# google/telluride_decoding

Hardware: AMD Instinct MI355X
Metric: TRF-fit samples/sec (higher is better)
Workload: dtype f32 (every product as 3 float16 products of a 2-piece split on the f16 MFMA, f32 accumulate, f64 slab sums; f64 solve)

## Files before the change

telluride_decoding_amd/csrc/lagcov.hip:

```cpp
#include <cstdlib>
#include <cstring>

#include "lag_common.h"

namespace {

constexpr int kTile = 128;
constexpr int kTileG = 64;
constexpr int kNpfU = 10;
constexpr int kNpfU2 = 13;
constexpr int kNpfG = 9;
constexpr int kLagsPerWg = 8;
constexpr int kHalo = 8;
constexpr size_t kLagcovScratchCap = size_t(256) << 20;

__device__ __forceinline__ int xcd_remap(int bid, int nwg) {
  const int q = nwg >> 3, r = nwg & 7;
  const int xcd = bid & 7, within = bid >> 3;
  const int base = xcd < r ? xcd * (q + 1) : r * (q + 1) + (xcd - r) * q;
  return base + within;
}

struct RowWindow {
  const float* base;
// ... 57 lines not shown
  v.y = (ok && c4 + 1 <= rw.last) ? v.y : 0.f;
  v.z = (ok && c4 + 2 <= rw.last) ? v.z : 0.f;
  v.w = (ok && c4 + 3 <= rw.last) ? v.w : 0.f;
  return v;
}

template <bool kUnified, int kTileT, int kNPF, bool kVec4>
__device__ __forceinline__ void prefetch_tile(const LagParams& p, const LagWork& w, long long ut,
                                              int e0, int rows, int cat, int cbt, int tid,
                                              float4 (&pf)[kNPF]) {
  const int c4 = (tid & 15) * 4;
  const int r0 = tid >> 4;
  if (kUnified) {
    const RowWindow rw = row_window(p.a, p.lda, w.a_row0, ut, w.a_valid, cat * 64, p.ca);
#pragma unroll
    for (int i = 0; i < kNPF; ++i) {
      const int r = r0 + 16 * i;
      pf[i] = load_row4<kVec4>(rw, r, r < rows, c4);
    }
  } else {
    const RowWindow ra = row_window(p.a, p.lda, w.a_row0, ut, w.a_valid, cat * 64, p.ca);
    const RowWindow rb = row_window(p.b, p.ldb, w.b_row0, ut + e0, w.b_valid, cbt * 64, p.cb);
    const long long a_left = w.u_end - ut;
    const int a_lim = (int)(a_left < kTileT ? a_left : kTileT);
#pragma unroll
    for (int i = 0; i < kNPF; ++i) {
      const int r = r0 + 16 * i;
      if (16 * i + 15 < kTileT)
        pf[i] = load_row4<kVec4>(ra, r, r < a_lim, c4);
      else
        pf[i] = load_row4<kVec4>(rb, r - kTileT, r < rows, c4);
    }
  }
}

template <bool kUnified, int kTileT, int kNPF>
__device__ __forceinline__ void store_tile(float* lds, const LagWork& w, long long ut,
                                           int ones_col, int tid, float4 (&pf)[kNPF]) {
  const int c4 = (tid & 15) * 4;
#pragma unroll
  for (int i = 0; i < kNPF; ++i) {
    const int r = (tid >> 4) + 16 * i;
    float4 v = pf[i];
    if (!kUnified && 16 * i + 15 < kTileT && ones_col >= c4 && ones_col < c4 + 4) {
      const long long u = ut + r;
      const float one = (u >= w.u_begin && u < w.u_end) ? 1.f : 0.f;
      if (ones_col == c4) v.x = one;
      else if (ones_col == c4 + 1) v.y = one;
      else if (ones_col == c4 + 2) v.z = one;
      else v.w = one;
    }
    *reinterpret_cast<float4*>(lds + r * 64 + c4) = v;
  }
}

template <int kTileT, bool kM2, bool kN2>
__device__ __forceinline__ void mfma_tile(const float* __restrict__ as,
                                          const float* __restrict__ bs, int wave, int lane, int nk,
                                          f32x16 (&acc)[2][2][2]) {
  const int lr = lane & 31, lk = lane >> 5;
  const float* ap = as + lk * 64 + lr;
  const float* bp = bs + (lk + 2 * wave) * 64 + lr;
  auto ld = [&](int kk, float (&o)[6]) {
    o[0] = ap[kk * 128];
    o[1] = kM2 ? ap[kk * 128 + 32] : 0.f;
    o[2] = bp[kk * 128];
    o[3] = kN2 ? bp[kk * 128 + 32] : 0.f;
    o[4] = bp[kk * 128 + 64];
    o[5] = kN2 ? bp[kk * 128 + 96] : 0.f;
  };
  auto mm = [&](const float (&o)[6]) {
#pragma unroll
    for (int le = 0; le < 2; ++le) {
      const float b0 = o[2 + 2 * le], b1 = o[3 + 2 * le];
      acc[le][0][0] = __builtin_amdgcn_mfma_f32_32x32x2f32(o[0], b0, acc[le][0][0], 0, 0, 0);
      if (kM2) acc[le][1][0] = __builtin_amdgcn_mfma_f32_32x32x2f32(o[1], b0, acc[le][1][0], 0, 0, 0);
      if (kN2) {
        acc[le][0][1] = __builtin_amdgcn_mfma_f32_32x32x2f32(o[0], b1, acc[le][0][1], 0, 0, 0);
        if (kM2) acc[le][1][1] = __builtin_amdgcn_mfma_f32_32x32x2f32(o[1], b1, acc[le][1][1], 0, 0, 0);
      }
    }
  };
  const int nfull = nk >> 1;
  float c[6], n[6];
  ld(0, c);
  int kk = 0;
  for (; kk + 1 < nfull; kk += 2) {
    ld(kk + 1, n);
    mm(c);
    ld(kk + 2 < nfull ? kk + 2 : kk + 1, c);
    mm(n);
  }
  if (kk < nfull) mm(c);
  if (nk & 1) {
    ld(nfull, c);
    if (lk) { c[0] = 0.f; c[1] = 0.f; }
    mm(c);
  }
}

template <int kTileT, bool kM2, bool kN2>
__device__ __forceinline__ void mfma_tile_few(const float* __restrict__ as,
                                              const float* __restrict__ bs, int wave, int lane,
                                              int nk, int g, int lg, f32x16 (&acc)[2][2][2]) {
  const int lr = lane & 31, lk = lane >> 5;
  const int s_phases = 8 >> lg;
  const int nfull = nk >> 1;
#pragma unroll
  for (int le = 0; le < 2; ++le) {
    const int slot = 2 * wave + le;
    const int lag = slot & (g - 1), phase = slot >> lg;
    const float* ap = as + lk * 64 + lr;
    const float* bp = bs + (lk + lag) * 64 + lr;
    auto step = [&](int kk, bool tail) {
      const bool live = !tail || lk == 0;
      const float a0 = live ? ap[kk * 128] : 0.f;
      const float a1 = (kM2 && live) ? ap[kk * 128 + 32] : 0.f;
      const float b0 = bp[kk * 128];
      acc[le][0][0] = __builtin_amdgcn_mfma_f32_32x32x2f32(a0, b0, acc[le][0][0], 0, 0, 0);
      if (kM2) acc[le][1][0] = __builtin_amdgcn_mfma_f32_32x32x2f32(a1, b0, acc[le][1][0], 0, 0, 0);
      if (kN2) {
        const float b1 = bp[kk * 128 + 32];
        acc[le][0][1] = __builtin_amdgcn_mfma_f32_32x32x2f32(a0, b1, acc[le][0][1], 0, 0, 0);
        if (kM2) acc[le][1][1] = __builtin_amdgcn_mfma_f32_32x32x2f32(a1, b1, acc[le][1][1], 0, 0, 0);
      }
    };
#pragma unroll 4
    for (int kk = phase; kk < nfull; kk += s_phases) step(kk, false);
    if ((nk & 1) && (nfull & (s_phases - 1)) == phase) step(nfull, true);
  }
}

template <bool kUnified, int kTileT, int kNPF, bool kVec4, bool kFew>
__global__ __launch_bounds__(kThreads, 2) void lagcov_mfma_kernel(LagParams p) {
  extern __shared__ __attribute__((aligned(16))) float lds[];

  const int tid = threadIdx.x;
  const int lane = tid & 63;
  const int wave = __builtin_amdgcn_readfirstlane(tid >> 6);

  int id = xcd_remap(blockIdx.x, gridDim.x);
  const int group = id % p.n_groups; id /= p.n_groups;
  const int cbt = id % p.n_cbt; id /= p.n_cbt;
  const int cat = id % p.n_cat; id /= p.n_cat;
  const LagWork w = p.works[id];
  const int e0 = p.e_min + group * (kFew ? p.lag_g : kLagsPerWg);

  const int rows = kUnified ? kTileT + kHalo + e0 : 2 * kTileT + kHalo;
  const float* as = lds;
  const float* bs = kUnified ? lds + e0 * 64 : lds + kTileT * 64;

  const int ca_eff = p.ca + p.a_ones;
  const bool m2 = ca_eff - cat * 64 > 32;
  const bool n2 = p.cb - cbt * 64 > 32;
  const int ones_col = p.a_ones ? p.ca - cat * 64 : -1;

  f32x16 acc[2][2][2];
#pragma unroll
  for (int i = 0; i < 2; ++i)
#pragma unroll
    for (int j = 0; j < 2; ++j)
#pragma unroll
      for (int k = 0; k < 2; ++k)
#pragma unroll
        for (int r = 0; r < 16; ++r) acc[i][j][k][r] = 0.f;

  float4 pf[kNPF];
  prefetch_tile<kUnified, kTileT, kNPF, kVec4>(p, w, w.u_begin, e0, rows, cat, cbt, tid, pf);
  store_tile<kUnified, kTileT, kNPF>(lds, w, w.u_begin, ones_col, tid, pf);
  __syncthreads();

  for (long long ut = w.u_begin; ut < w.u_end; ut += kTileT) {
    const bool more = ut + kTileT < w.u_end;
    if (more)
      prefetch_tile<kUnified, kTileT, kNPF, kVec4>(p, w, ut + kTileT, e0, rows, cat, cbt, tid,
                                                      pf);
    const long long left = w.u_end - ut;
    const int nk = (kUnified && left < kTileT) ? (int)left : kTileT;
    if (kFew) {
      if (m2) {
        if (n2) mfma_tile_few<kTileT, true, true>(as, bs, wave, lane, nk, p.lag_g, p.lag_lg, acc);
        else    mfma_tile_few<kTileT, true, false>(as, bs, wave, lane, nk, p.lag_g, p.lag_lg, acc);
      } else {
        if (n2) mfma_tile_few<kTileT, false, true>(as, bs, wave, lane, nk, p.lag_g, p.lag_lg, acc);
        else    mfma_tile_few<kTileT, false, false>(as, bs, wave, lane, nk, p.lag_g, p.lag_lg, acc);
      }
    } else if (m2) {
      if (n2) mfma_tile<kTileT, true, true>(as, bs, wave, lane, nk, acc);
      else    mfma_tile<kTileT, true, false>(as, bs, wave, lane, nk, acc);
    } else {
      if (n2) mfma_tile<kTileT, false, true>(as, bs, wave, lane, nk, acc);
      else    mfma_tile<kTileT, false, false>(as, bs, wave, lane, nk, acc);
    }
    if (more) {
      __syncthreads();
      store_tile<kUnified, kTileT, kNPF>(lds, w, ut + kTileT, ones_col, tid, pf);
      __syncthreads();
    }
  }

  const int lr = lane & 31, lk = lane >> 5;
  float* slab = p.partial + (size_t)id * p.e_pad * p.ca_pad * p.cb_pad;
#pragma unroll
  for (int le = 0; le < 2; ++le) {
    int e_idx = group * kLagsPerWg + 2 * wave + le;
    if (kFew) {
      const int slot = 2 * wave + le;
      e_idx = ((slot >> p.lag_lg) * p.n_groups + group) * p.lag_g + (slot & (p.lag_g - 1));
    }
    float* pe = slab + (size_t)e_idx * p.ca_pad * p.cb_pad;
#pragma unroll
    for (int m = 0; m < 2; ++m)
#pragma unroll
      for (int n = 0; n < 2; ++n)
#pragma unroll
        for (int r = 0; r < 16; ++r) {
          const int i = cat * 64 + m * 32 + (r & 3) + 8 * (r >> 2) + 4 * lk;
          const int j = cbt * 64 + n * 32 + lr;
          pe[(size_t)i * p.cb_pad + j] = acc[le][m][n][r];
        }
  }
}

constexpr int kBfTile = 128;
template <int kRowDw, int kPieces> struct BfGeom {
  static constexpr int kRows = kRowDw == 83 ? 160 : 192;
  static constexpr int kPieceDw = 64 * kRowDw;
  static constexpr size_t kLdsBytes =
      sizeof(unsigned) * (2 * kPieces * kPieceDw + (kPieces == 2 ? 2 * 2 * 96 + 8 * 1024 : 0));
};
constexpr int kBfThreads = 512;

typedef td_u32x4 u32x4;

__device__ __forceinline__ float comp4(const float4& v, int q) {
  return q == 0 ? v.x : q == 1 ? v.y : q == 2 ? v.z : v.w;
}

#define TD_KS_C0(r) "0"
#define TD_KS_C1(r) "%" #r
#define TD_KS_BODY(C, MASK_L, MASK_H, TAIL)                                              \
  "ds_read2_b32 v[224:225], %[bp0] offset0:%[o0] offset1:%[o1]\n"                        \
  "ds_read2_b32 v[226:227], %[bp0] offset0:%[o2] offset1:%[o3]\n"                        \
  "ds_read2_b32 v[228:229], %[bp0] offset0:%[o4] offset1:%[o5]\n"                        \
  "ds_read_b32 v230, %[bp0] offset:%[ob]\n"                                              \
  "ds_read2_b32 v[220:221], %[ap1] offset0:%[o0] offset1:%[o1]\n"                        \
  "ds_read2_b32 v[222:223], %[ap1] offset0:%[o2] offset1:%[o3]\n"                        \
  "ds_read2_b32 v[232:233], %[bp1] offset0:%[o0] offset1:%[o1]\n"                        \
  "ds_read2_b32 v[234:235], %[bp1] offset0:%[o2] offset1:%[o3]\n"                        \
  "ds_read2_b32 v[236:237], %[bp1] offset0:%[o4] offset1:%[o5]\n"                        \
  "ds_read_b32 v238, %[bp1] offset:%[ob]\n"                                              \
  "ds_read2_b32 v[216:217], %[ap0] offset0:%[o0] offset1:%[o1]\n"                        \
  "ds_read2_b32 v[218:219], %[ap0] offset0:%[o2] offset1:%[o3]\n"                        \
  "s_waitcnt lgkmcnt(6)\n"                                                               \
  MASK_L                                                                                 \
  "v_alignbit_b32 v240, v225, v224, 16\n"                                                \
  "v_alignbit_b32 v241, v226, v225, 16\n"                                                \
  "v_alignbit_b32 v242, v227, v226, 16\n"                                                \
  "v_alignbit_b32 v243, v228, v227, 16\n"                                                \
  "v_alignbit_b32 v244, v229, v228, 16\n"                                                \
  "v_alignbit_b32 v245, v230, v229, 16\n"                                                \
  "v_mfma_f32_32x32x16_f16 %0, v[220:223], v[224:227], " C(0) "\n"                       \
  "s_waitcnt lgkmcnt(0)\n"                                                               \
  MASK_H                                                                                 \
  "v_alignbit_b32 v248, v233, v232, 16\n"                                                \
  "v_alignbit_b32 v249, v234, v233, 16\n"                                                \
  "v_mfma_f32_32x32x16_f16 %1, v[220:223], v[240:243], " C(1) "\n"                       \
  "v_alignbit_b32 v250, v235, v234, 16\n"                                                \
  "v_alignbit_b32 v251, v236, v235, 16\n"                                                \
  "v_mfma_f32_32x32x16_f16 %2, v[220:223], v[226:229], " C(2) "\n"                       \
  "v_alignbit_b32 v252, v237, v236, 16\n"                                                \
  "v_alignbit_b32 v253, v238, v237, 16\n"                                                \
  "v_mfma_f32_32x32x16_f16 %3, v[220:223], v[242:245], " C(3) "\n"                       \
  "v_mfma_f32_32x32x16_f16 %0, v[216:219], v[232:235], %0\n"                             \
  "v_mfma_f32_32x32x16_f16 %1, v[216:219], v[248:251], %1\n"                             \
  "v_mfma_f32_32x32x16_f16 %2, v[216:219], v[234:237], %2\n"                             \
  "v_mfma_f32_32x32x16_f16 %3, v[216:219], v[250:253], %3\n"                             \
  "v_mfma_f32_32x32x16_f16 %0, v[216:219], v[224:227], %0\n"                             \
  "v_mfma_f32_32x32x16_f16 %1, v[216:219], v[240:243], %1\n"                             \
  "v_mfma_f32_32x32x16_f16 %2, v[216:219], v[226:229], %2\n"                             \
  "v_mfma_f32_32x32x16_f16 %3, v[216:219], v[242:245], %3\n"                             \
  TAIL
#define TD_KS_MASK_L                                                                     \
  "v_and_b32 v220, %[m0], v220\n" "v_and_b32 v221, %[m1], v221\n"                        \
  "v_and_b32 v222, %[m2], v222\n" "v_and_b32 v223, %[m3], v223\n"
#define TD_KS_MASK_H                                                                     \
  "v_and_b32 v216, %[m0], v216\n" "v_and_b32 v217, %[m1], v217\n"                        \
  "v_and_b32 v218, %[m2], v218\n" "v_and_b32 v219, %[m3], v219\n"
#define TD_KS_TAIL "s_nop 15\ns_nop 3\n"
#define TD_KS_INS                                                                        \
  [ap0] "v"(ap0), [ap1] "v"(ap1), [bp0] "v"(bp0), [bp1] "v"(bp1),                        \
  [o0] "n"(kOff), [o1] "n"(kOff + 1), [o2] "n"(kOff + 2), [o3] "n"(kOff + 3),            \
  [o4] "n"(kOff + 4), [o5] "n"(kOff + 5), [ob] "n"(4 * (kOff + 6)),                      \
  [m0] "v"(m0), [m1] "v"(m1), [m2] "v"(m2), [m3] "v"(m3)
#define TD_KS_CLOBBER                                                                    \
  "memory", "v216", "v217", "v218", "v219", "v220", "v221", "v222", "v223", "v224", "v225", "v226", "v227", \
  "v228", "v229", "v230", "v231", "v232", "v233", "v234", "v235", "v236", "v237", "v238", "v239", "v240",   \
  "v241", "v242", "v243", "v244", "v245", "v246", "v247", "v248", "v249", "v250", "v251", "v252", "v253",   \
  "v254", "v255"
#define TD_KS_ASM(OUT, C, ML, MH, TAIL)                                                  \
  asm volatile(TD_KS_BODY(C, ML, MH, TAIL)                                               \
               : OUT(acc[0]), OUT(acc[1]), OUT(acc[2]), OUT(acc[3]) : TD_KS_INS : TD_KS_CLOBBER)

__device__ __forceinline__ unsigned lds_addr(const unsigned* p) {
  return (unsigned)(size_t)(__attribute__((address_space(3))) const unsigned*)p;
}

template <bool kZero, bool kMask, bool kLast, int kOff>
__device__ __forceinline__ void bf_kstep_skip(unsigned ap0, unsigned ap1, unsigned bp0, unsigned bp1,
                                              const unsigned* a_mask, f32x16 (&acc)[4]) {
  unsigned m0 = 0, m1 = 0, m2 = 0, m3 = 0;
  if constexpr (kMask) { m0 = a_mask[0]; m1 = a_mask[1]; m2 = a_mask[2]; m3 = a_mask[3]; }
  if constexpr (kZero) {
    if constexpr (kMask) {
      if constexpr (kLast) TD_KS_ASM("=&v", TD_KS_C0, TD_KS_MASK_L, TD_KS_MASK_H, TD_KS_TAIL);
      else TD_KS_ASM("=&v", TD_KS_C0, TD_KS_MASK_L, TD_KS_MASK_H, "");
    } else {
      if constexpr (kLast) TD_KS_ASM("=&v", TD_KS_C0, "", "", TD_KS_TAIL);
      else TD_KS_ASM("=&v", TD_KS_C0, "", "", "");
    }
  } else {
    if constexpr (kMask) {
      if constexpr (kLast) TD_KS_ASM("+v", TD_KS_C1, TD_KS_MASK_L, TD_KS_MASK_H, TD_KS_TAIL);
      else TD_KS_ASM("+v", TD_KS_C1, TD_KS_MASK_L, TD_KS_MASK_H, "");
    } else {
      if constexpr (kLast) TD_KS_ASM("+v", TD_KS_C1, "", "", TD_KS_TAIL);
      else TD_KS_ASM("+v", TD_KS_C1, "", "", "");
    }
  }
}

template <bool kZero, int kBfPieceDw, bool kF16, bool kSkip = false, int kOff = 0, bool kLast = true>
__device__ __forceinline__ void bf_kstep(const unsigned* __restrict__ ap,
                                         const unsigned* __restrict__ bp,
                                         const unsigned* a_mask, f32x16 (&acc)[4]) {
  if constexpr (kSkip) {
    static_assert(kF16, "lags +0, +1, +4, +5: the float16 form");
    const unsigned a0 = lds_addr(ap), b0 = lds_addr(bp);
    if (a_mask) bf_kstep_skip<kZero, true, kLast, kOff>(a0, a0 + 4 * kBfPieceDw, b0, b0 + 4 * kBfPieceDw, a_mask, acc);
    else bf_kstep_skip<kZero, false, kLast, kOff>(a0, a0 + 4 * kBfPieceDw, b0, b0 + 4 * kBfPieceDw, a_mask, acc);
    return;
  }
  constexpr int kP = kF16 ? 2 : 3;
  u32x4 a[kP];
  unsigned d[kP][6];
#pragma unroll
  for (int pc = 0; pc < kP; ++pc) {
#pragma unroll
    for (int i = 0; i < 4; ++i) a[pc][i] = ap[pc * kBfPieceDw + i];
#pragma unroll
    for (int i = 0; i < 6; ++i) d[pc][i] = bp[pc * kBfPieceDw + i];
  }
  if (a_mask) {
#pragma unroll
    for (int pc = 0; pc < kP; ++pc)
#pragma unroll
      for (int i = 0; i < 4; ++i) a[pc][i] &= a_mask[i];
  }
  u32x4 b[4][kP];
#pragma unroll
  for (int pc = 0; pc < kP; ++pc)
#pragma unroll
    for (int i = 0; i < 4; ++i) {
      b[0][pc][i] = d[pc][i];
      b[1][pc][i] = __builtin_amdgcn_alignbit(d[pc][i + 1], d[pc][i], 16);
      b[2][pc][i] = d[pc][i + 1];
      b[3][pc][i] = __builtin_amdgcn_alignbit(d[pc][i + 2], d[pc][i + 1], 16);
    }
  f32x16 c[4];
#pragma unroll
  for (int r = 0; r < 4; ++r) {
    if (kZero) {
#pragma unroll
      for (int k = 0; k < 16; ++k) c[r][k] = 0.f;
    } else {
      c[r] = acc[r];
    }
  }
  if constexpr (kF16) {
    constexpr int pa[3] = {1, 0, 0}, pb[3] = {0, 1, 0};
#pragma unroll
    for (int t = 0; t < 3; ++t)
#pragma unroll
      for (int r = 0; r < 4; ++r) c[r] = td_mfma_f16(a[pa[t] % kP], b[r][pb[t] % kP], c[r]);
  } else {
    constexpr int pa[6] = {2, 0, 1, 1, 0, 0}, pb[6] = {0, 2, 1, 0, 1, 0};
#pragma unroll
    for (int t = 0; t < 6; ++t)
#pragma unroll
      for (int r = 0; r < 4; ++r) c[r] = td_mfma_bf16(a[pa[t] % kP], b[r][pb[t] % kP], c[r]);
  }
#pragma unroll
  for (int r = 0; r < 4; ++r) acc[r] = c[r];
}

template <int kFrom, int kTo, int kBfPieceDw, bool kF16, int kChain, bool kSkip = false>
__device__ __forceinline__ void bf_ksteps(const unsigned* __restrict__ ap,
                                          const unsigned* __restrict__ bp, f32x16 (&acc)[4],
                                          f32x16 (&total)[4]) {
  if constexpr (kSkip) {
    if constexpr (kFrom < kTo) {
      constexpr bool kLast = (kFrom + 1) % kChain == 0;
      bf_kstep<kFrom % kChain == 0, kBfPieceDw, kF16, true, 8 * kFrom, kLast>(ap, bp, nullptr, acc);
      if (kLast) {
#pragma unroll
        for (int r = 0; r < 4; ++r) total[r] += acc[r];
      }
      __builtin_amdgcn_sched_barrier(0);
      bf_ksteps<kFrom + 1, kTo, kBfPieceDw, kF16, kChain, true>(ap, bp, acc, total);
    }
    return;
  }
#pragma unroll
  for (int s = kFrom; s < kTo; ++s) {
    if (s % kChain == 0) bf_kstep<true, kBfPieceDw, kF16>(ap + 8 * s, bp + 8 * s, nullptr, acc);
    else                 bf_kstep<false, kBfPieceDw, kF16>(ap + 8 * s, bp + 8 * s, nullptr, acc);
    if ((s + 1) % kChain == 0) {
#pragma unroll
      for (int r = 0; r < 4; ++r) total[r] += acc[r];
    }
    __builtin_amdgcn_sched_barrier(0);
  }
}

template <bool kVec4, int kBfRowDw, bool kF16, bool kVirt = false, bool kKs = false>
__global__ __launch_bounds__(kBfThreads) void lagcov_split_kernel(LagParams p) {
  static_assert(!kVirt || kF16, "virtual images: the float16 form");
  static_assert(!kKs || kVirt, "shared tasks: virtual images");
  constexpr int kChain = 8;
  constexpr int kP = kF16 ? 2 : 3;
  extern __shared__ __attribute__((aligned(16))) unsigned ldsu[];
  constexpr int kBfRows = BfGeom<kBfRowDw, kP>::kRows;
  constexpr int kBfPieceDw = BfGeom<kBfRowDw, kP>::kPieceDw;

  const int tid = threadIdx.x;
  const int lane = tid & 63;
  const int wave = __builtin_amdgcn_readfirstlane(tid >> 6);
  int quad = wave & 1, mt = (wave >> 1) & 1, nt = wave >> 2;
  constexpr bool kSkip = kF16 && !kVirt;

  int id = xcd_remap(blockIdx.x, gridDim.x);
  const int group = id % p.n_groups; id /= p.n_groups;
  const int part = id;
  LagWork w = p.works[id];
  const int e0 = group * kLagsPerWg;
  int lag_off = e0 + (kSkip ? 2 : 4) * quad, out_lag = lag_off;
  bool active = true, a_ext = false;
  const VirtImage* img = nullptr;
  VirtSeg vs = {0, 0, 0};
  int kparts = 1, kq = 0;
  if constexpr (kVirt) {
    const VirtGroup* vg = p.vgroups + group;
    const VirtTask tk = vg->task[wave];
    img = p.vimgs + vg->image;
    mt = tk.mt; nt = tk.nt; lag_off = tk.lag0; out_lag = tk.out_lag;
    active = out_lag >= 0; a_ext = tk.a_ext != 0;
    if constexpr (kKs) {
      kparts = __builtin_amdgcn_readfirstlane((int)tk.kparts);
      kq = __builtin_amdgcn_readfirstlane((int)tk.kq);
    }
    vs = p.vsegs[id];
  }
  const int ksn = 8 / kparts, ks0 = kq * ksn;

  f32x16 total[4];
#pragma unroll
  for (int r = 0; r < 4; ++r)
#pragma unroll
    for (int k = 0; k < 16; ++k) total[r][k] = 0.f;

  const int c4 = (tid & 15) * 4, rg = tid >> 4;
  const bool has_tail = kBfRows == 192 || wave < 4;
  const bool early = wave < 4;
  float sc[4] = {1.f, 1.f, 1.f, 1.f};
  int vdesc[4] = {0, 0, 0, 0};
  if constexpr (kVirt) {
#pragma unroll
    for (int q = 0; q < 4; ++q) {
      const int k = kVec4 ? c4 + q : lane;
      vdesc[q] = (img->src[k] + 1) | (img->role[k] ? 0x100 : 0) | ((int)img->shift[k] << 16);
    }
  }
  constexpr int kVPairs = kBfRows / 16;
  auto v_src = [&](int q) { return (vdesc[q] & 0xff) - 1; };
  auto v_sh = [&](int q) { return vdesc[q] >> 16; };
  auto v_role = [&](int q) { return (vdesc[q] & 0x100) != 0; };
  if (kF16) {
#pragma unroll
    for (int q = 0; q < 4; ++q) {
      const int ch = kVirt ? v_src(q) : min(c4 + q, 63);
      const int k = ch >= 0 ? td_f16_scale_exp(td_chan_max_of(p.chan_max, ch)) : 0;
      sc[q] = __builtin_bit_cast(float, (unsigned)(127 + k) << 23);
      if (kVirt && ch < 0) sc[q] = 0.f;
    }
    if (blockIdx.x == 0 && tid < 128) {
      unsigned* all = const_cast<unsigned*>(p.chan_max);
      const unsigned m = td_chan_max_of(p.chan_max, tid);
      all[kChanShards * 128 + tid] = m;
      if (p.scale_out) p.scale_out[tid] = m;
    }
    if (p.zero_tab && blockIdx.x == (gridDim.x > 1 ? 1 : 0))
      for (int i = tid; i < kChanTab; i += kBfThreads) p.zero_tab[i] = 0u;
  }
  const bool never = false;
  float anchor_a = 0.f, anchor_b = 1.f;
  auto sched_anchor = [&](unsigned* dst) {
    if (!never || tid >= 160) return;
    reinterpret_cast<unsigned short*>(dst)[tid] = (unsigned short)(anchor_a * anchor_b);
  };
  float4 pf[6];
  auto interior = [&](long long ut) -> bool {
    return kVec4 && p.ca == 64 && ut >= 0 && ut + kBfRows <= w.a_valid;
  };
  auto vrange = [&](long long ut, int q, int& lo, int& hi) {
    const long long lim = 1 << 20;
    const long long a0 = -ut, b0 = w.a_valid - ut;
    const long long a1 = vs.seg_begin - ut, b1 = (vs.seg_end < w.a_valid ? vs.seg_end : w.a_valid) - ut;
    const int a0i = (int)(a0 < -lim ? -lim : (a0 > lim ? lim : a0)), b0i = (int)(b0 < -lim ? -lim : (b0 > lim ? lim : b0));
    const int a1i = (int)(a1 < -lim ? -lim : (a1 > lim ? lim : a1)), b1i = (int)(b1 < -lim ? -lim : (b1 > lim ? lim : b1));
    lo = (v_role(q) ? a1i : a0i) - v_sh(q);
    hi = (v_role(q) ? b1i : b0i) - v_sh(q);
    if (v_src(q) < 0) { lo = 0; hi = 0; }
  };
  int v_min_shift = 0, v_max_shift = 0;
  bool v_any_role1 = false;
  if constexpr (kVirt) { v_min_shift = img->min_shift; v_max_shift = img->max_shift; v_any_role1 = img->any_role1 != 0; }
  auto vinside = [&](long long ut) -> bool {
    const long long lo = v_any_role1 && vs.seg_begin > 0 ? vs.seg_begin : 0;
    const long long hi = v_any_role1 && vs.seg_end < w.a_valid ? vs.seg_end : w.a_valid;
    return ut + v_min_shift >= lo && ut + kBfRows + v_max_shift <= hi;
  };
  auto prefetch_to = [&](long long ut, float4 (&pfr)[6]) {
    if constexpr (kVirt) {
      if (vinside(ut)) {
        const int ld = (int)p.lda;
        const float* base = p.a + (w.a_row0 + ut) * p.lda;
        if (kVec4) {
          const int off = (4 * rg + v_sh(0)) * ld + (v_src(0) < 0 ? 0 : v_src(0));
#pragma unroll
          for (int s = 0; s < 4; ++s) pfr[s] = *reinterpret_cast<const float4*>(base + s * ld + off);
          if (has_tail) {
            const float* tb = base + kBfTile * ld;
            const int toff = off - 2 * rg * ld;
#pragma unroll
            for (int s = 0; s < 2; ++s) pfr[4 + s] = *reinterpret_cast<const float4*>(tb + s * ld + toff);
          }
        } else {
          const int off = (2 * wave + v_sh(0)) * ld + (v_src(0) < 0 ? 0 : v_src(0));
          float* pv = reinterpret_cast<float*>(&pfr[0]);
#pragma unroll
          for (int j = 0; j < kVPairs; ++j) {
            pv[2 * j] = (base + 16 * j * ld)[off];
            pv[2 * j + 1] = (base + (16 * j + 1) * ld)[off];
          }
        }
        return;
      }
      const float* base = p.a + (w.a_row0 + ut) * p.lda;
      const int ld = (int)p.lda;
      const long long l0 = -ut, h0 = w.a_valid - 1 - ut, lim = 1 << 20;
      const int rlo = (int)(l0 < -lim ? -lim : (l0 > lim ? lim : l0));
      const int rhi = (int)(h0 < -lim ? -lim : (h0 > lim ? lim : h0));
      if (kVec4) {
        const int src = v_src(0) < 0 ? 0 : v_src(0), sh = v_sh(0);
#pragma unroll
        for (int s = 0; s < 4; ++s) {
          const int rc = max(rlo, min(4 * rg + s + sh, rhi));
          pfr[s] = *reinterpret_cast<const float4*>(base + rc * ld + src);
        }
        if (has_tail) {
#pragma unroll
          for (int s = 0; s < 2; ++s) {
            const int rc = max(rlo, min(kBfTile + 2 * rg + s + sh, rhi));
            pfr[4 + s] = *reinterpret_cast<const float4*>(base + rc * ld + src);
          }
        }
      } else {
        const int src = v_src(0) < 0 ? 0 : v_src(0), sh = v_sh(0);
        float* pv = reinterpret_cast<float*>(&pfr[0]);
#pragma unroll
        for (int j = 0; j < 2 * kVPairs; ++j) {
          const int r = 16 * (j >> 1) + 2 * wave + (j & 1);
          const int rc = max(rlo, min(r + sh, rhi));
          pv[j] = base[rc * ld + src];
        }
      }
      return;
    }
    if (interior(ut)) {
      const float* base = p.a + (w.a_row0 + ut) * p.lda + c4;
      const int ld = (int)p.lda;
#pragma unroll
      for (int s = 0; s < 4; ++s)
        pfr[s] = *reinterpret_cast<const float4*>(base + (4 * rg + s) * ld);
      if (has_tail) {
#pragma unroll
        for (int s = 0; s < 2; ++s)
          pfr[4 + s] = *reinterpret_cast<const float4*>(base + (kBfTile + 2 * rg + s) * ld);
      }
      return;
    }
    const RowWindow rw = row_window(p.a, p.lda, w.a_row0, ut, w.a_valid, 0, p.ca);
#pragma unroll
    for (int s = 0; s < 4; ++s) pfr[s] = load_row4_raw<kVec4>(rw, 4 * rg + s, c4);
    if (has_tail) {
#pragma unroll
      for (int s = 0; s < 2; ++s) pfr[4 + s] = load_row4_raw<kVec4>(rw, kBfTile + 2 * rg + s, c4);
    }
  };
  auto prefetch = [&](long long ut) { prefetch_to(ut, pf); };
  auto store_from = [&](long long ut, unsigned* buf, const float4 (&pfr)[6]) {
    if constexpr (kVirt && !kVec4) {
      const float* pv = reinterpret_cast<const float*>(&pfr[0]);
      unsigned* dst = buf + lane * kBfRowDw + wave;
      if (vinside(ut)) {
#pragma unroll
        for (int j = 0; j < kVPairs; ++j) {
          unsigned h, l;
          td_split2_f16(pv[2 * j] * sc[0], pv[2 * j + 1] * sc[0], h, l);
          dst[8 * j] = h;
          dst[kBfPieceDw + 8 * j] = l;
        }
        return;
      }
      int lo, hi;
      vrange(ut, 0, lo, hi);
#pragma unroll
      for (int j = 0; j < kVPairs; ++j) {
        const int r = 16 * j + 2 * wave;
        const float x0 = (r >= lo && r < hi) ? pv[2 * j] : 0.f;
        const float x1 = (r + 1 >= lo && r + 1 < hi) ? pv[2 * j + 1] : 0.f;
        unsigned h, l;
        td_split2_f16(x0 * sc[0], x1 * sc[0], h, l);
        dst[8 * j] = h;
        dst[kBfPieceDw + 8 * j] = l;
      }
      return;
    }
    float4 vcopy[6];
    float4 (&v)[6] = kSkip ? const_cast<float4 (&)[6]>(pfr) : vcopy;
    if constexpr (!kSkip) {
#pragma unroll
      for (int s = 0; s < 6; ++s) vcopy[s] = pfr[s];
    }
    if constexpr (kVirt) {
      if (!vinside(ut))
#pragma unroll
      for (int q = 0; q < 4; ++q) {
        int lo, hi;
        vrange(ut, kVec4 ? 0 : q, lo, hi);
        if (lo <= 0 && hi >= kBfRows) continue;
#pragma unroll
        for (int s = 0; s < 4; ++s) {
          const int r = 4 * rg + s;
          float& x = reinterpret_cast<float*>(&v[s])[q];
          x = (r >= lo && r < hi) ? x : 0.f;
        }
#pragma unroll
        for (int s = 0; s < 2; ++s) {
          const int r = kBfTile + 2 * rg + s;
          float& x = reinterpret_cast<float*>(&v[4 + s])[q];
          x = (r >= lo && r < hi) ? x : 0.f;
        }
      }
    } else
    if (!interior(ut)) {
      const RowWindow rw = row_window(p.a, p.lda, w.a_row0, ut, w.a_valid, 0, p.ca);
#pragma unroll
      for (int s = 0; s < 4; ++s) v[s] = mask_row4(rw, 4 * rg + s, true, c4, pfr[s]);
      if (has_tail) {
#pragma unroll
        for (int s = 0; s < 2; ++s) v[4 + s] = mask_row4(rw, kBfTile + 2 * rg + s, true, c4, pfr[4 + s]);
      }
    }
#pragma unroll
    for (int q = 0; q < 4; ++q) {
      unsigned* dst = buf + (c4 + q) * kBfRowDw + 2 * rg;
      if (kF16) {
        unsigned h[2], l[2];
#pragma unroll
        for (int d = 0; d < 2; ++d)
          td_split2_f16(comp4(v[2 * d], q) * sc[q], comp4(v[2 * d + 1], q) * sc[q], h[d], l[d]);
        dst[0] = h[0]; dst[1] = h[1];
        dst[kBfPieceDw] = l[0]; dst[kBfPieceDw + 1] = l[1];
      } else {
        unsigned h[2], m[2], l[2];
#pragma unroll
        for (int d = 0; d < 2; ++d)
          td_split3(comp4(v[2 * d], q), comp4(v[2 * d + 1], q), h[d], m[d], l[d]);
        dst[0] = h[0]; dst[1] = h[1];
        dst[kBfPieceDw] = m[0]; dst[kBfPieceDw + 1] = m[1];
        dst[(kP - 1) * kBfPieceDw] = l[0]; dst[(kP - 1) * kBfPieceDw + 1] = l[1];
      }
    }
    if (has_tail) {
#pragma unroll
      for (int q = 0; q < 4; ++q) {
        unsigned* tail = buf + (c4 + q) * kBfRowDw + kBfTile / 2 + rg;
        if (kF16) {
          unsigned h, l;
          td_split2_f16(comp4(v[4], q) * sc[q], comp4(v[5], q) * sc[q], h, l);
          tail[0] = h;
          tail[kBfPieceDw] = l;
        } else {
          unsigned h, m, l;
          td_split3(comp4(v[4], q), comp4(v[5], q), h, m, l);
          tail[0] = h;
          tail[kBfPieceDw] = m;
          tail[(kP - 1) * kBfPieceDw] = l;
        }
      }
    }
  };
// ... 1579 lines not shown
```

Measured before the change: 1.164 billion.

## Fuse consecutive skip-path k-steps into one software-pipelined inline-asm run

Replaces the per-k-step inline asm on the float16 skip path with multi-step asm blocks (runs of 2 or 4 k-steps). These double-buffer the LDS operand registers, so the reads for the next step are issued while the current step's MFMAs run, using graded lgkmcnt waits. The aim is to hide LDS latency and drop the per-step s_nop tail and sched barriers between steps. The masked single-step variant is kept only for the non-zero, last-step case, which adds hand-managed register and wait-count complexity.

New measurement: 1.178 billion, median of 6. +1.2%, better.

```diff
diff --git a/telluride_decoding_amd/csrc/lagcov.hip b/telluride_decoding_amd/csrc/lagcov.hip
--- a/telluride_decoding_amd/csrc/lagcov.hip
+++ b/telluride_decoding_amd/csrc/lagcov.hip
@@ -383,43 +383,92 @@
   asm volatile(TD_KS_BODY(C, ML, MH, TAIL)                                               \
                : OUT(acc[0]), OUT(acc[1]), OUT(acc[2]), OUT(acc[3]) : TD_KS_INS : TD_KS_CLOBBER)
 
+#define TD_KP_RD_A(D, P, K)                                                              \
+  "ds_read2_b32 v[" #D ":" #D "+1], " P " offset0:%[k0]+" #K " offset1:%[k0]+" #K "+1\n"     \
+  "ds_read2_b32 v[" #D "+2:" #D "+3], " P " offset0:%[k0]+" #K "+2 offset1:%[k0]+" #K "+3\n"
+#define TD_KP_RD_B(D, P, K)                                                              \
+  TD_KP_RD_A(D, P, K)                                                                    \
+  "ds_read2_b32 v[" #D "+4:" #D "+5], " P " offset0:%[k0]+" #K "+4 offset1:%[k0]+" #K "+5\n" \
+  "ds_read_b32 v[" #D "+6], " P " offset:%[kb]+4*" #K "\n"
+#define TD_KP_HEAD                                                                       \
+  TD_KP_RD_B(224, "%[bp0]", 0) TD_KP_RD_A(220, "%[ap1]", 0)                              \
+  TD_KP_RD_B(232, "%[bp1]", 0) TD_KP_RD_A(216, "%[ap0]", 0)
+#define TD_KP_Q(D, Q)                                                                    \
+  "v_alignbit_b32 v[" #Q "], v[" #D "+1], v[" #D "], 16\n"                               \
+  "v_alignbit_b32 v[" #Q "+1], v[" #D "+2], v[" #D "+1], 16\n"                           \
+  "v_alignbit_b32 v[" #Q "+2], v[" #D "+3], v[" #D "+2], 16\n"                           \
+  "v_alignbit_b32 v[" #Q "+3], v[" #D "+4], v[" #D "+3], 16\n"                           \
+  "v_alignbit_b32 v[" #Q "+4], v[" #D "+5], v[" #D "+4], 16\n"                           \
+  "v_alignbit_b32 v[" #Q "+5], v[" #D "+6], v[" #D "+5], 16\n"
+#define TD_KP_MFMA(r, A, B, I, C)                                                        \
+  "v_mfma_f32_32x32x16_f16 %" #r ", " A ", v[" #B "+" #I ":" #B "+" #I "+3], " C "\n"
+#define TD_KP_STEP(C, HD, HQ, LD, LQ, RD_AL, W, RD_BH, RD_BL_AH)                         \
+  "s_waitcnt lgkmcnt(6)\n"                                                               \
+  TD_KP_MFMA(0, "v[220:223]", HD, 0, C(0))                                               \
+  TD_KP_Q(HD, HQ)                                                                        \
+  TD_KP_MFMA(1, "v[220:223]", HQ, 0, C(1))                                               \
+  TD_KP_MFMA(2, "v[220:223]", HD, 2, C(2))                                               \
+  TD_KP_MFMA(3, "v[220:223]", HQ, 2, C(3))                                               \
+  RD_AL                                                                                  \
+  "s_waitcnt lgkmcnt(" #W ")\n"                                                          \
+  TD_KP_MFMA(0, "v[216:219]", LD, 0, "%0")                                               \
+  TD_KP_Q(LD, LQ)                                                                        \
+  TD_KP_MFMA(1, "v[216:219]", LQ, 0, "%1")                                               \
+  TD_KP_MFMA(2, "v[216:219]", LD, 2, "%2")                                               \
+  TD_KP_MFMA(3, "v[216:219]", LQ, 2, "%3")                                               \
+  RD_BH                                                                                  \
+  TD_KP_MFMA(0, "v[216:219]", HD, 0, "%0")                                               \
+  TD_KP_MFMA(1, "v[216:219]", HQ, 0, "%1")                                               \
+  TD_KP_MFMA(2, "v[216:219]", HD, 2, "%2")                                               \
+  TD_KP_MFMA(3, "v[216:219]", HQ, 2, "%3")                                               \
+  RD_BL_AH
+#define TD_KP_EVEN(C, K)                                                                 \
+  TD_KP_STEP(C, 224, 240, 232, 248, TD_KP_RD_A(220, "%[ap1]", K), 2,                     \
+             TD_KP_RD_B(232, "%[bp0]", K), TD_KP_RD_B(224, "%[bp1]", K) TD_KP_RD_A(216, "%[ap0]", K))
+#define TD_KP_ODD(C, K)                                                                  \
+  TD_KP_STEP(C, 232, 248, 224, 240, TD_KP_RD_A(220, "%[ap1]", K), 2,                     \
+             TD_KP_RD_B(224, "%[bp0]", K), TD_KP_RD_B(232, "%[bp1]", K) TD_KP_RD_A(216, "%[ap0]", K))
+#define TD_KP_ODD_END(C) TD_KP_STEP(C, 232, 248, 224, 240, "", 0, "", "")
+#define TD_KP_RUN2(C) TD_KP_HEAD TD_KP_EVEN(C, 8) TD_KP_ODD_END(TD_KS_C1)
+#define TD_KP_RUN4 TD_KP_HEAD TD_KP_EVEN(TD_KS_C1, 8) TD_KP_ODD(TD_KS_C1, 16) TD_KP_EVEN(TD_KS_C1, 24) TD_KP_ODD_END(TD_KS_C1)
+#define TD_KP_ASM(OUT, BODY)                                                             \
+  asm volatile(BODY : OUT(acc[0]), OUT(acc[1]), OUT(acc[2]), OUT(acc[3])                 \
+               : [ap0] "v"(ap0), [ap1] "v"(ap1), [bp0] "v"(bp0), [bp1] "v"(bp1),         \
+                 [k0] "n"(kOff), [kb] "n"(4 * (kOff + 6)) : TD_KS_CLOBBER)
+
 __device__ __forceinline__ unsigned lds_addr(const unsigned* p) {
   return (unsigned)(size_t)(__attribute__((address_space(3))) const unsigned*)p;
 }
 
-template <bool kZero, bool kMask, bool kLast, int kOff>
+template <int kOff = 0>
 __device__ __forceinline__ void bf_kstep_skip(unsigned ap0, unsigned ap1, unsigned bp0, unsigned bp1,
                                               const unsigned* a_mask, f32x16 (&acc)[4]) {
-  unsigned m0 = 0, m1 = 0, m2 = 0, m3 = 0;
-  if constexpr (kMask) { m0 = a_mask[0]; m1 = a_mask[1]; m2 = a_mask[2]; m3 = a_mask[3]; }
-  if constexpr (kZero) {
-    if constexpr (kMask) {
-      if constexpr (kLast) TD_KS_ASM("=&v", TD_KS_C0, TD_KS_MASK_L, TD_KS_MASK_H, TD_KS_TAIL);
-      else TD_KS_ASM("=&v", TD_KS_C0, TD_KS_MASK_L, TD_KS_MASK_H, "");
-    } else {
-      if constexpr (kLast) TD_KS_ASM("=&v", TD_KS_C0, "", "", TD_KS_TAIL);
-      else TD_KS_ASM("=&v", TD_KS_C0, "", "", "");
-    }
+  const unsigned m0 = a_mask[0], m1 = a_mask[1], m2 = a_mask[2], m3 = a_mask[3];
+  TD_KS_ASM("+v", TD_KS_C1, TD_KS_MASK_L, TD_KS_MASK_H, TD_KS_TAIL);
+}
+
+template <bool kZero, bool kLast, int kSteps, int kOff>
+__device__ __forceinline__ void bf_krun_skip(unsigned ap0, unsigned ap1, unsigned bp0, unsigned bp1,
+                                             f32x16 (&acc)[4]) {
+  static_assert(kSteps == 2 || (kSteps == 4 && !kZero && !kLast), "the runs of a tile: 2, 4, 2 k-steps");
+  if constexpr (kSteps == 4) TD_KP_ASM("+v", TD_KP_RUN4);
+  else if constexpr (kZero) {
+    if constexpr (kLast) TD_KP_ASM("=&v", TD_KP_RUN2(TD_KS_C0) TD_KS_TAIL);
+    else TD_KP_ASM("=&v", TD_KP_RUN2(TD_KS_C0));
   } else {
-    if constexpr (kMask) {
-      if constexpr (kLast) TD_KS_ASM("+v", TD_KS_C1, TD_KS_MASK_L, TD_KS_MASK_H, TD_KS_TAIL);
-      else TD_KS_ASM("+v", TD_KS_C1, TD_KS_MASK_L, TD_KS_MASK_H, "");
-    } else {
-      if constexpr (kLast) TD_KS_ASM("+v", TD_KS_C1, "", "", TD_KS_TAIL);
-      else TD_KS_ASM("+v", TD_KS_C1, "", "", "");
-    }
-  }
-}
-
-template <bool kZero, int kBfPieceDw, bool kF16, bool kSkip = false, int kOff = 0, bool kLast = true>
+    if constexpr (kLast) TD_KP_ASM("+v", TD_KP_RUN2(TD_KS_C1) TD_KS_TAIL);
+    else TD_KP_ASM("+v", TD_KP_RUN2(TD_KS_C1));
+  }
+}
+
+template <bool kZero, int kBfPieceDw, bool kF16, bool kSkip = false>
 __device__ __forceinline__ void bf_kstep(const unsigned* __restrict__ ap,
                                          const unsigned* __restrict__ bp,
                                          const unsigned* a_mask, f32x16 (&acc)[4]) {
   if constexpr (kSkip) {
-    static_assert(kF16, "lags +0, +1, +4, +5: the float16 form");
+    static_assert(kF16 && !kZero, "lags +0, +1, +4, +5: the float16 form, a masked step onto zeroed sums");
     const unsigned a0 = lds_addr(ap), b0 = lds_addr(bp);
-    if (a_mask) bf_kstep_skip<kZero, true, kLast, kOff>(a0, a0 + 4 * kBfPieceDw, b0, b0 + 4 * kBfPieceDw, a_mask, acc);
-    else bf_kstep_skip<kZero, false, kLast, kOff>(a0, a0 + 4 * kBfPieceDw, b0, b0 + 4 * kBfPieceDw, a_mask, acc);
+    bf_kstep_skip(a0, a0 + 4 * kBfPieceDw, b0, b0 + 4 * kBfPieceDw, a_mask, acc);
     return;
   }
   constexpr int kP = kF16 ? 2 : 3;
@@ -480,16 +529,16 @@
                                           const unsigned* __restrict__ bp, f32x16 (&acc)[4],
                                           f32x16 (&total)[4]) {
   if constexpr (kSkip) {
-    if constexpr (kFrom < kTo) {
-      constexpr bool kLast = (kFrom + 1) % kChain == 0;
-      bf_kstep<kFrom % kChain == 0, kBfPieceDw, kF16, true, 8 * kFrom, kLast>(ap, bp, nullptr, acc);
-      if (kLast) {
-#pragma unroll
-        for (int r = 0; r < 4; ++r) total[r] += acc[r];
-      }
-      __builtin_amdgcn_sched_barrier(0);
-      bf_ksteps<kFrom + 1, kTo, kBfPieceDw, kF16, kChain, true>(ap, bp, acc, total);
-    }
+    static_assert(kF16 && kFrom / kChain == (kTo - 1) / kChain, "a run lies within one MFMA chain");
+    constexpr bool kLast = kTo % kChain == 0;
+    const unsigned a0 = lds_addr(ap), b0 = lds_addr(bp);
+    bf_krun_skip<kFrom % kChain == 0, kLast, kTo - kFrom, 8 * kFrom>(a0, a0 + 4 * kBfPieceDw, b0,
+                                                                     b0 + 4 * kBfPieceDw, acc);
+    if (kLast) {
+#pragma unroll
+      for (int r = 0; r < 4; ++r) total[r] += acc[r];
+    }
+    __builtin_amdgcn_sched_barrier(0);
     return;
   }
 #pragma unroll
```
